# nv-tlabs/ChronoEdit

Hardware: AMD Instinct MI355X
Metric: denoising-steps/sec (higher is better)
Workload: dtype bf16

## Files before the change

chronoedit_amd/csrc/ce_common.h:

```cpp
#pragma once
#include <hip/hip_runtime.h>
#include <stdint.h>

typedef __bf16 bf16;
typedef __attribute__((ext_vector_type(2))) __bf16 bf16x2;
typedef __attribute__((ext_vector_type(4))) __bf16 bf16x4;
typedef __attribute__((ext_vector_type(8))) __bf16 bf16x8;
typedef __attribute__((ext_vector_type(2))) float f32x2;
typedef __attribute__((ext_vector_type(4))) float f32x4;
typedef __attribute__((ext_vector_type(16))) float f32x16;
typedef __attribute__((ext_vector_type(4))) uint32_t u32x4;
typedef __attribute__((ext_vector_type(2))) uint32_t u32x2;

#define CE_WAVE 64

#define CE_API extern "C" __attribute__((visibility("default")))
#ifdef CE_DIAGNOSTICS
#define CE_KNOB static int
#define CE_DIAG_COUNT_EXACT(counter)                                        \
  do {                                                                      \
    if ((threadIdx.x & 63) == 0) atomicAdd(&(counter), 1ull);               \
  } while (0)
#else
#define CE_KNOB static constexpr int
// ... 7 lines not shown

#define CE_MAX_DEVICES 16
inline int ce_device_slot() {
  int d = 0;
  if (hipGetDevice(&d) != hipSuccess || d < 0 || d >= CE_MAX_DEVICES) d = 0;
  return d;
}

inline int ce_device_cus() {
  static int cus_[CE_MAX_DEVICES] = {};
  int& cus = cus_[ce_device_slot()];
  if (cus == 0) {
    int dev = 0, n = 0;
    cus = (hipGetDevice(&dev) == hipSuccess && hipDeviceGetAttribute(&n, hipDeviceAttributeMultiprocessorCount, dev) == hipSuccess && n > 0) ? n : 256;
  }
  return cus;
}

inline int ce_split_k(int tail, int kt, int cus, long long slab_bytes, long long ws_bytes) {
  if (tail <= 0) return 1;
  for (int s = cus / tail < 8 ? cus / tail : 8; s >= 2; --s)
    if (kt % (2 * s) == 0 && tail * s * slab_bytes <= ws_bytes) return s;
  return 1;
}

inline uint32_t ce_seg_magic(int seg_k, int bk, int kt) {
  if (seg_k <= 0 || seg_k % bk) return 0;
  const int tps = seg_k / bk;
  const uint32_t magic = 65536u / (uint32_t)tps + 1u;
  for (int t = 0; t < kt; ++t)
    if ((int)((uint32_t)t * magic >> 16) != t / tps) return 0;
  return magic;
}

__device__ __forceinline__ float bf16_bits_to_f32(uint32_t bits16) { return __uint_as_float(bits16 << 16); }
__device__ __forceinline__ float bf16lo(uint32_t packed) { return __uint_as_float(packed << 16); }
__device__ __forceinline__ float bf16hi(uint32_t packed) { return __uint_as_float(packed & 0xffff0000u); }

__device__ __forceinline__ uint32_t pack_bf16(float lo, float hi) {
  f32x2 v = {lo, hi};
  bf16x2 r = __builtin_convertvector(v, bf16x2);
  return __builtin_bit_cast(uint32_t, r);
}
__device__ __forceinline__ float round_bf16(float x) {
  bf16 b = (bf16)x;
  return (float)b;
// ... 60 lines not shown
```

chronoedit_amd/csrc/ce_gemm.hip:

```cpp
#include <cmath>

#include "ce_common.h"

#define EPI_BIAS 0
#define EPI_BIAS_GELU 1
#define EPI_GATE_RES 2
#define EPI_BIAS_GELU_ERF 3
#define EPI_F32 4
#define EPI_BIAS_ROW 6
#define EPI_BIAS_T 7
#define EPI_MUL 5

namespace {

constexpr int BM = 128, BN = 128, BK = 64;
constexpr int TILE_BYTES = BM * BK * 2;
constexpr int LDC_BYTES = BN * 2 + 16;

__device__ __forceinline__ int swz_chunk(int row, int chunk) { return chunk ^ ((row >> 1) & 7); }

template <int EPI>
__global__ __launch_bounds__(256) void gemm_bf16_128(const bf16* __restrict__ A, const bf16* __restrict__ W,
                                                     bf16* __restrict__ C, const float* __restrict__ bias,
                                                     const float* __restrict__ gate, const bf16* __restrict__ res, int M,
// ... 179 lines not shown
                                 hipStream_t stream);

extern "C" void ce_gemm256_set_staggered(int on);
extern "C" int ce_gemm384_launch(const void* A, const void* W, void* C, const float* bias, int epilogue, const float* gate,
                                 const void* res, int M, int N, int K, int lda, int ldw, int ldc, int ldres, int gate_rows, int res_rows,
                                 int a_seg_k, long long a_seg_stride, int w_seg_k, long long w_seg_stride, float* ws, size_t ws_bytes,
                                 hipStream_t stream);
extern "C" int ce_gemm288_launch(const void* A, const void* W, void* C, const float* bias, int epilogue, const float* gate,
                                 const void* res, int M, int N, int K, int lda, int ldw, int ldc, int ldres, int gate_rows, int res_rows,
                                 int a_seg_k, long long a_seg_stride, int w_seg_k, long long w_seg_stride, float* ws, size_t ws_bytes,
                                 hipStream_t stream);
extern "C" int ce_gemm256w4_launch(const void* A, const void* W, void* C, const float* bias, int epilogue, const float* gate,
                                   const void* res, int M, int N, int K, int lda, int ldw, int ldc, int ldres, int gate_rows, int res_rows,
                                   int a_seg_k, long long a_seg_stride, int w_seg_k, long long w_seg_stride, int nsa, float* ws,
                                   size_t ws_bytes, hipStream_t stream);

CE_KNOB g_gemm_variant = -1;
#ifdef CE_DIAGNOSTICS
CE_API int ce_set_gemm_variant(int v) {
  const int old = g_gemm_variant;
  g_gemm_variant = v;
  ce_gemm256_set_staggered(v == 2);
  return old;
}
#endif

CE_API int ce_gemm_bf16_tile_rows(int M, int N, int K, int cus, long long ws_bytes) {
  if (M <= 0 || N <= 0 || K < 64 || cus <= 0) return 0;
  const int kt = K / 64;
  auto cost = [&](int bm) -> double {
    const long long nwg = (long long)((M + bm - 1) / bm) * ((N + 255) / 256);
    const long long full = nwg / cus;
    const int tail = (int)(nwg % cus);
    const double llc = (double)M * K * 2.0 > 128.0 * 1048576.0 ? 1.04 : 1.0;
    const double c = bm == 256 ? 1.40 : bm == 288 ? 1.40 * 1.125 * 0.985 * llc : 1.40 * 1.5 * 0.96 * llc;
    double t = (double)full * kt * c;
    if (tail > 0) {
      const int split = ce_split_k(tail, kt, cus, bm * 256 * (long long)sizeof(float), ws_bytes);
      if (split > 1) t += (double)kt / split * c + (double)tail * split * bm * 256.0 * 8.0 / 6.0e6;
      else t += (double)kt * c * pow((double)tail / cus, 0.3);
    }
    return t;
  };
  const double c384 = cost(384), c256 = cost(256);
  if (M % 288 == 0) {
    const long long nwg = (long long)(M / 288) * ((N + 255) / 256);
// ... 112 lines not shown
```

chronoedit_amd/csrc/ce_gemm256w4.hip:

```cpp
#include "ce_common.h"
#include "ce_gemm_epi.h"

namespace {

constexpr int BM = 256, BN = 256, BK = 64;
constexpr int TILE = 256 * BK * 2;
constexpr int CROW = BN * 2 + 16;
constexpr int QROW = 128 * 2 + 16;

typedef __attribute__((address_space(3))) void lds_void;

#define W4_VM(N) asm volatile("s_waitcnt vmcnt(" #N ")" ::: "memory")
#define W4_LGKM0() asm volatile("s_waitcnt lgkmcnt(0)" ::: "memory")
#define W4_BAR() __builtin_amdgcn_s_barrier()
#define W4_PIN() __builtin_amdgcn_sched_barrier(0)

__device__ __forceinline__ void tile_origin_w4(int wg, int tiles_m, int tiles_n, int bn, int& m0, int& n0) {
  constexpr int GROUP = 4;
  const int group_sz = GROUP * tiles_n;
  const int gid = wg / group_sz;
  const int first_m = gid * GROUP;
  const int gm = min(tiles_m - first_m, GROUP);
  m0 = (first_m + (wg % group_sz) % gm) * BM;
  n0 = ((wg % group_sz) / gm) * bn;
}

template <int NG>
struct FragSet {
  bf16x8 a[8], b[NG];
};

#define W4_MMA(F, G, S)                                                                                                      \
  if ((G) < NG) {                                                                                                            \
    if constexpr (REGEPI)                                                                                                    \
      asm volatile("v_mfma_f32_16x16x32_bf16 %0, %1, %2, %0" : "+a"(acc[F][(G) < NG ? (G) : 0]) : "v"((S).a[F]), "v"((S).b[(G) < NG ? (G) : 0])); \
    else                                                                                                                     \
      asm volatile("v_mfma_f32_16x16x32_bf16 %0, %1, %2, %0" : "+a"(acc[F][(G) < NG ? (G) : 0]) : "v"((S).b[(G) < NG ? (G) : 0]), "v"((S).a[F])); \
  }

template <int EPI, int NSA, bool ONEBAR, bool SEG2 = false, int NG = 8>
__global__ __launch_bounds__(256) __attribute__((amdgpu_waves_per_eu(1, 1))) void gemm_bf16_w4(
    const bf16* __restrict__ A, const bf16* __restrict__ W, bf16* __restrict__ C, const float* __restrict__ bias,
    const float* __restrict__ gate, const bf16* __restrict__ res, int M, int N, int K, int lda, int ldw, int ldc, int ldres,
    int gate_rows, int res_rows, int tiles_m, int tiles_n, int t_full, int split, float* __restrict__ ws, uint32_t a_seg_magic,
    uint32_t a_seg_extra, uint32_t w_seg_magic, uint32_t w_seg_extra, uint32_t a_seg2_magic, uint32_t a_seg2_extra) {
  extern __shared__ __attribute__((aligned(16))) unsigned char smem[];
  constexpr int BN = 32 * NG;
  constexpr bool REGEPI = NG == 8;
  constexpr int NW = NG;
  constexpr int WTILE = BN * BK * 2;
  constexpr int CROW = BN * 2 + 16;
  constexpr int W_RING = NSA * TILE;
  const int tid = threadIdx.x, lane = tid & 63;
  const int wave = __builtin_amdgcn_readfirstlane(tid >> 6);
  const int wm = wave >> 1, wn = wave & 1;
  const int fr = lane & 15, fg = lane >> 4;

  const bool partial = (int)blockIdx.x >= t_full;
  int wg, kt0 = 0, ktn = K / BK;
  if (!partial) {
    wg = xcd_remap(blockIdx.x, t_full);
  } else {
    const int tb = blockIdx.x - t_full;
    wg = t_full + tb / split;
    ktn = ktn / split;
    kt0 = (tb % split) * ktn;
  }
  int m0, n0;
  tile_origin_w4(wg, tiles_m, tiles_n, BN, m0, n0);
  const int kt_last = ktn - 1;

  uint32_t a_voff[8], w_voff[8];
#pragma unroll
  for (int p = 0; p < 8; ++p) {
    const int row = 8 * (wave + 4 * p) + (lane >> 3);
    const int chunk = (lane & 7) ^ ((row >> 1) & 7);
    a_voff[p] = (uint32_t)min(m0 + row, M - 1) * (uint32_t)(lda * 2) + chunk * 16;
    const int wrow = REGEPI ? ((row & 128) | ((row & 15) << 3) | ((row & 127) >> 4)) : row;
    w_voff[p] = (uint32_t)min(n0 + wrow, N - 1) * (uint32_t)(ldw * 2) + chunk * 16;
  }
  const auto a_rsrc = __builtin_amdgcn_make_buffer_rsrc((void*)A, 0, 0xffffffffu, 0x00020000);
  const auto w_rsrc = __builtin_amdgcn_make_buffer_rsrc((void*)W, 0, 0xffffffffu, 0x00020000);
  auto koff = [&](int t, uint32_t magic, uint32_t extra) __attribute__((always_inline)) -> int {
    const int ta = kt0 + min(t, kt_last);
    return ta * (BK * 2) + (int)((((uint32_t)ta * magic) >> 16) * extra);
  };
  auto koff_a = [&](int t) __attribute__((always_inline)) -> int {
    int o = koff(t, a_seg_magic, a_seg_extra);
    if (SEG2) o += (int)((((uint32_t)(kt0 + min(t, kt_last)) * a_seg2_magic) >> 16) * a_seg2_extra);
    return o;
  };
  auto dma_a = [&](int p, int stage_bytes, int soff) __attribute__((always_inline)) {
    __builtin_amdgcn_raw_ptr_buffer_load_lds(a_rsrc, (lds_void*)(smem + stage_bytes + (wave + 4 * p) * 1024), 16, a_voff[p], soff, 0, 0);
  };
  auto dma_w = [&](int p, int stage_bytes, int soff) __attribute__((always_inline)) {
    if (p < NW)
      __builtin_amdgcn_raw_ptr_buffer_load_lds(w_rsrc, (lds_void*)(smem + W_RING + stage_bytes + (wave + 4 * p) * 1024), 16, w_voff[p < NW ? p : 0], soff, 0, 0);
  };

  int a_rd[2], w_rd[2];
#pragma unroll
  for (int ks = 0; ks < 2; ++ks) {
    a_rd[ks] = (wm * 128 + fr) * 128 + (((fg + 4 * ks) ^ (fr >> 1)) << 4);
    w_rd[ks] = W_RING + (wn * (BN / 2) + fr) * 128 + (((fg + 4 * ks) ^ (fr >> 1)) << 4);
  }
  auto read_frag = [&](int r, int a_stage_bytes, int w_stage_bytes, FragSet<NG>& k0, FragSet<NG>& k1) __attribute__((always_inline)) {
    FragSet<NG>& s = (r >> 4) ? k1 : k0;
    const int ks = r >> 4, f = r & 7;
    if (((r >> 3) & 1) == 0)
      s.a[f] = *reinterpret_cast<const bf16x8*>(smem + a_rd[ks] + a_stage_bytes + f * 2048);
    else if (f < NG)
      s.b[f < NG ? f : 0] = *reinterpret_cast<const bf16x8*>(smem + w_rd[ks] + w_stage_bytes + f * 2048);
  };

  f32x4 acc[8][NG];
#pragma unroll
  for (int f = 0; f < 8; ++f)
#pragma unroll
    for (int g = 0; g < NG; ++g) acc[f][g] = f32x4{0.f, 0.f, 0.f, 0.f};

  {
    const int a0 = koff_a(0), w0 = koff(0, w_seg_magic, w_seg_extra);
    const int a1 = koff_a(1), w1 = koff(1, w_seg_magic, w_seg_extra);
#pragma unroll
    for (int p = 0; p < 8; ++p) dma_a(p, 0, a0);
#pragma unroll
    for (int p = 0; p < 8; ++p) dma_w(p, 0, w0);
#pragma unroll
    for (int p = 0; p < 8; ++p) dma_a(p, TILE, a1);
#pragma unroll
    for (int p = 0; p < 8; ++p) dma_w(p, WTILE, w1);
    if (NSA == 3 && !ONEBAR) {
      const int a2 = koff_a(2);
#pragma unroll
      for (int p = 0; p < 8; ++p) dma_a(p, 2 * TILE, a2);
    }
  }
  if (NSA == 3 && !ONEBAR) W4_VM(24); else if (NG == 8) W4_VM(16); else if (NG == 4) W4_VM(12); else W4_VM(11);
  W4_BAR();
  FragSet<NG> s0, s1, s2;
#pragma unroll
  for (int r = 0; r < 32; ++r) read_frag(r, 0, 0, s0, s1);
  W4_LGKM0();
  W4_PIN();

  int a_st = 0;
#define W4_TILE(T, WP, K0, K1, KN)                                                                              \
  {                                                                                                             \
    const int a_next = (a_st + TILE == NSA * TILE) ? 0 : a_st + TILE;                                          \
    const int a_nn = (a_next + TILE == NSA * TILE) ? 0 : a_next + TILE;                                        \
    const int wsoff = koff((T) + 2, w_seg_magic, w_seg_extra);                                                 \
    const int asoff = koff_a((T) + (ONEBAR ? 2 : NSA));                                                        \
    const int a_dst = ONEBAR ? a_nn : a_st;                                                                     \
    if (!ONEBAR) W4_BAR();                                                                                      \
    W4_UNIT0(0, K0, WP, wsoff) W4_UNIT0(1, K0, WP, wsoff) W4_UNIT0(2, K0, WP, wsoff) W4_UNIT0(3, K0, WP, wsoff) \
    W4_UNIT0(4, K0, WP, wsoff) W4_UNIT0(5, K0, WP, wsoff) W4_UNIT0(6, K0, WP, wsoff) W4_UNIT0(7, K0, WP, wsoff) \
    if (NSA == 3 && !ONEBAR) W4_VM(16); else if (NG == 8) W4_VM(8); else if (NG == 4) W4_VM(4); else W4_VM(3);   \
    W4_BAR();                                                                                                   \
    W4_UNIT1(0, K1, K0, KN, WP) W4_UNIT1(1, K1, K0, KN, WP) W4_UNIT1(2, K1, K0, KN, WP) W4_UNIT1(3, K1, K0, KN, WP) \
    W4_UNIT1(4, K1, K0, KN, WP) W4_UNIT1(5, K1, K0, KN, WP) W4_UNIT1(6, K1, K0, KN, WP) W4_UNIT1(7, K1, K0, KN, WP) \
    W4_LGKM0();                                                                                                 \
    W4_PIN();                                                                                                   \
    a_st = a_next;                                                                                              \
  }
#define W4_UNIT0(F, K0, WP, WSOFF)                                                                                 \
  W4_MMA(F, 0, K0);                                                                                                \
  if (ONEBAR) dma_a(F, a_dst, asoff); else dma_w(F, (WP) * WTILE, WSOFF);                                          \
  W4_PIN();                                                                                                        \
  W4_MMA(F, 1, K0); W4_MMA(F, 2, K0); W4_MMA(F, 3, K0); W4_MMA(F, 4, K0); W4_MMA(F, 5, K0); W4_MMA(F, 6, K0);      \
  W4_MMA(F, 7, K0); W4_PIN();
#define W4_UNIT1(F, K1, K0, KN, WP)                                                                                \
  W4_MMA(F, 0, K1);                                                                                                \
  if (ONEBAR) dma_w(F, (WP) * WTILE, wsoff); else dma_a(F, a_dst, asoff);                                          \
  W4_PIN();                                                                                                        \
  W4_MMA(F, 1, K1); W4_PIN();                                                                                      \
  W4_MMA(F, 2, K1); read_frag(4 * (F) + 0, a_next, (1 - (WP)) * WTILE, K0, KN); W4_PIN();                           \
  W4_MMA(F, 3, K1); read_frag(4 * (F) + 1, a_next, (1 - (WP)) * WTILE, K0, KN); W4_PIN();                           \
  W4_MMA(F, 4, K1); read_frag(4 * (F) + 2, a_next, (1 - (WP)) * WTILE, K0, KN); W4_PIN();                           \
  W4_MMA(F, 5, K1); read_frag(4 * (F) + 3, a_next, (1 - (WP)) * WTILE, K0, KN); W4_PIN();                           \
  W4_MMA(F, 6, K1); W4_MMA(F, 7, K1); W4_PIN();

  const int npairs = ktn >> 1;
  for (int it = 0; it < npairs; ++it) {
    const int t = 2 * it;
    W4_TILE(t, 0, s0, s1, s2)
    W4_TILE(t + 1, 1, s0, s2, s1)
  }
#undef W4_TILE
#undef W4_UNIT0
#undef W4_UNIT1
  W4_VM(0);
  W4_LGKM0();
  asm volatile("s_nop 15\n\ts_nop 15" ::: "memory");
  static_assert(NG == 8 || ((NG == 4 || NG == 3) && NSA == 2 && !ONEBAR), "the 256 x 128 / 256 x 96 tiles exist for the two-stage loop only");
  if constexpr (REGEPI) {
    const int col0 = n0 + wn * 128 + fr * 8;
    const bool col_ok = col0 < N;
    const int colc = min(col0, N - 8);
    const int row_base = m0 + wm * 128 + fg * 4;
    if (partial) {
      float* slab = ws + (size_t)(blockIdx.x - t_full) * (BM * BN);
#pragma unroll
      for (int f = 0; f < 8; ++f) {
        f32x4 av[8];
#pragma unroll
        for (int g = 0; g < 8; ++g) {
          asm volatile("" : "+a"(acc[f][g]));
          av[g] = acc[f][g];
        }
#pragma unroll
        for (int jj = 0; jj < 4; ++jj)
#pragma unroll
          for (int h = 0; h < 2; ++h) {
            const f32x4 o = {av[4 * h + 0][jj], av[4 * h + 1][jj], av[4 * h + 2][jj], av[4 * h + 3][jj]};
            const int lane_o = fg * 4 + jj + 16 * (2 * (fr & 1) + h);
            *reinterpret_cast<f32x4*>(slab + (((wave * 64 + f * 8 + (fr >> 1)) * 64) + lane_o) * 4) = o;
          }
      }
      return;
    }
    f32x4 bvv[2];
#pragma unroll
    for (int h = 0; h < 2; ++h)
      bvv[h] = (EPI != EPI_BIAS_ROW && bias != nullptr) ? *reinterpret_cast<const f32x4*>(bias + colc + 4 * h) : f32x4{0.f, 0.f, 0.f, 0.f};
    const auto c_rsrc = __builtin_amdgcn_make_buffer_rsrc((void*)C, 0, (uint32_t)(M - 1) * (uint32_t)(ldc * 2) + (uint32_t)N * 2u, 0x00020000);
    f32x4 gA[2], gB[2];
    int g_switch = 0x7fffffff;
    u32x4 rv[8][4];
    if (EPI == EPI_GATE_RES) {
      gA[0] = gA[1] = gB[0] = gB[1] = f32x4{1.f, 1.f, 1.f, 1.f};
      if (gate != nullptr) {
        const int s0 = gate_rows > 0 ? m0 / gate_rows : 0;
        const int s1 = gate_rows > 0 ? min(M - 1, m0 + BM - 1) / gate_rows : 0;
        const float* ga = gate + (size_t)s0 * N + colc;
        const float* gb = gate + (size_t)s1 * N + colc;
        gA[0] = *reinterpret_cast<const f32x4*>(ga);
        gA[1] = *reinterpret_cast<const f32x4*>(ga + 4);
        gB[0] = *reinterpret_cast<const f32x4*>(gb);
        gB[1] = *reinterpret_cast<const f32x4*>(gb + 4);
        if (s1 != s0) g_switch = s1 * gate_rows;
      }
#pragma unroll
      for (int f = 0; f < 8; ++f)
#pragma unroll
        for (int jj = 0; jj < 4; ++jj)
          rv[f][jj] = *reinterpret_cast<const u32x4*>(res + (size_t)res_row(min(row_base + f * 16 + jj, M - 1), res_wrap(m0, res_rows)) * ldres + colc);
    }
#pragma unroll
    for (int f = 0; f < 8; ++f) {
      f32x4 av[8];
#pragma unroll
      for (int g = 0; g < 8; ++g) {
        asm volatile("" : "+a"(acc[f][g]));
        av[g] = acc[f][g];
      }
      f32x4 brow4 = {0.f, 0.f, 0.f, 0.f};
      if (EPI == EPI_BIAS_ROW) brow4 = *reinterpret_cast<const f32x4*>(bias + min(row_base + f * 16, M - 4));
#pragma unroll
      for (int jj = 0; jj < 4; ++jj) {
        const int m = row_base + f * 16 + jj;
        u32x4 y;
#pragma unroll
        for (int q = 0; q < 4; ++q) {
          const int h = q >> 1, e = 2 * (q & 1);
          const float b0 = EPI == EPI_BIAS_ROW ? brow4[jj] : bvv[h][e], b1 = EPI == EPI_BIAS_ROW ? brow4[jj] : bvv[h][e + 1];
          y[q] = pack_bf16(av[2 * q][jj] + b0, av[2 * q + 1][jj] + b1);
        }
        u32x4 o = y;
        if (EPI == EPI_BIAS_GELU) {
#pragma unroll
          for (int q = 0; q < 4; ++q) o[q] = pack_bf16(gelu_tanh(bf16lo(y[q])), gelu_tanh(bf16hi(y[q])));
        } else if (EPI == EPI_BIAS_GELU_ERF) {
// ... 108 lines not shown
        const u32x4 r = rv[p][tt];
        u32x4 o;
#pragma unroll
        for (int q = 0; q < 4; ++q) {
          const float ga = q < 2 ? g0[2 * q] : g1[2 * q - 4], gb = q < 2 ? g0[2 * q + 1] : g1[2 * q - 3];
          o[q] = pack_bf16(mul_then_add(bf16lo(y[q]), ga, bf16lo(r[q])), mul_then_add(bf16hi(y[q]), gb, bf16hi(r[q])));
        }
        const uint32_t coff = (m < M && my_n < N) ? (uint32_t)m * (uint32_t)(ldc * 2) + (uint32_t)my_n * 2u : 0xffffffffu;
        __builtin_amdgcn_raw_buffer_store_b128(o, c_rsrc, coff, 0, 0);
      }
    } else if (EPI != EPI_GATE_RES) {
      epi_chunks<EPI, CH>(smem, CROW,
                         [&](int tt, int& rl, int& cc, int& mr) {
                           bool ok;
                           rl = chunk_row(tt, ok);
                           cc = my_cc;
                           mr = ok ? (rl >> 5) * 128 + p * 32 + (rl & 31) : (1 << 28);
                         },
                         m0, n0, C, gate, res, M, N, ldc, ldres, gate_rows, res_rows);
    }
  }
}

template <int EPI>
__global__ __launch_bounds__(256) void gemm256w4_reduce(bf16* __restrict__ C, const float* __restrict__ bias, const float* __restrict__ gate,
                                                        const bf16* __restrict__ res, int M, int N, int ldc, int ldres, int gate_rows, int res_rows,
                                                        int tiles_m, int tiles_n, int t_full, int split, const float* __restrict__ ws) {
  extern __shared__ __attribute__((aligned(16))) unsigned char smem[];
  const int tid = threadIdx.x, lane = tid & 63, w = tid >> 6;
  const int fr = lane & 15, fg = lane >> 4;
  const int tile = blockIdx.x >> 2, q = blockIdx.x & 3;
  int m0, n0;
  tile_origin_w4(t_full + tile, tiles_m, tiles_n, BN, m0, n0);
  m0 += (q >> 1) * 128;
  n0 += (q & 1) * 128;
  const float* slab = ws + (size_t)tile * split * (BM * BN);
#pragma unroll
  for (int ff = 0; ff < 2; ++ff) {
    const int f = 2 * w + ff;
    const int rl = f * 16 + fr;
    float brow = 0.f;
    if (EPI == EPI_BIAS_ROW) brow = bias[min(m0 + rl, M - 1)];
#pragma unroll
    for (int g = 0; g < 8; ++g) {
      const int cl = g * 16 + fg * 4;
      f32x4 bv = (EPI != EPI_BIAS_ROW && bias != nullptr) ? *reinterpret_cast<const f32x4*>(bias + min(n0 + cl, N - 4)) : f32x4{0.f, 0.f, 0.f, 0.f};
      if (EPI == EPI_BIAS_ROW) bv[0] = bv[1] = bv[2] = bv[3] = brow;
      const int e = (((q * 64 + f * 8 + g) * 64) + lane) * 4;
      f32x4 v = *reinterpret_cast<const f32x4*>(slab + e);
      for (int sidx = 1; sidx < split; ++sidx) v += *reinterpret_cast<const f32x4*>(slab + (size_t)sidx * (BM * BN) + e);
      const u32x2 pk = {pack_bf16(v[0] + bv[0], v[1] + bv[1]), pack_bf16(v[2] + bv[2], v[3] + bv[3])};
      *reinterpret_cast<u32x2*>(smem + rl * QROW + cl * 2) = pk;
    }
  }
  __syncthreads();
  epi_chunks<EPI, 8>(smem, QROW, [&](int tt, int& rl, int& cc, int& mr) { const int c = tid + 256 * tt; rl = mr = c >> 4; cc = c & 15; }, m0, n0,
                     C, gate, res, M, N, ldc, ldres, gate_rows, res_rows);
}

}

extern "C" int ce_gemm256_launch(const void* A, const void* W, void* C, const float* bias, int epilogue, const float* gate,
// ... 20 lines not shown
  const int tiles_m = (M + BM - 1) / BM, tiles_n = (N + bn - 1) / bn;
  const int nwg = tiles_m * tiles_n, kt = K / BK;
  uint32_t a_seg_magic = 0, a_seg_extra = 0, w_seg_magic = 0, w_seg_extra = 0;
  auto seg = [&](int seg_k, long long seg_stride, uint32_t& magic, uint32_t& extra_out) -> int {
    if (seg_k <= 0 || seg_k >= K) return CE_OK;
    magic = ce_seg_magic(seg_k, BK, kt);
    const long long extra = (seg_stride - seg_k) * 2;
    if (!magic || extra < 0 || extra * ((K + seg_k - 1) / seg_k) + (long long)K * 2 >= (1ll << 31)) return CE_ERR_SHAPE;
    extra_out = (uint32_t)extra;
    return CE_OK;
  };
  if (int rc = seg(a_seg_k, a_seg_stride, a_seg_magic, a_seg_extra)) return rc;
  if (int rc = seg(w_seg_k, w_seg_stride, w_seg_magic, w_seg_extra)) return rc;
  uint32_t a_seg2_magic = 0, a_seg2_extra = 0;
  if (seg2 && a_seg2_k < K) {
    a_seg2_magic = ce_seg_magic(a_seg2_k, BK, kt);
    if (!a_seg2_magic) return CE_ERR_SHAPE;
    const long long extra = (a_seg2_stride - (long long)(a_seg2_k / a_seg_k) * a_seg_stride) * 2;
    const long long reach = ((long long)(K - 1) / a_seg2_k) * a_seg2_stride * 2 + (long long)(a_seg2_k / a_seg_k) * a_seg_stride * 2 + (long long)a_seg_k * 2;
    if (extra < 0 || reach >= (1ll << 31)) return CE_ERR_SHAPE;
    a_seg2_extra = (uint32_t)extra;
  }
  const int cus = ce_device_cus();
  int tail = nwg % cus;
  const int split = seg2 ? 1 : ce_split_k(tail, kt, cus, BM * BN * sizeof(float), ws ? (long long)ws_bytes : 0);
  if (split == 1) tail = 0;
  const int t_full2 = nwg - tail;
  dim3 grid(t_full2 + tail * split), block(256);
  const int lds3 = 5 * TILE, lds2 = 4 * TILE;
  if (seg2) {
    const int lds2n = 2 * TILE + 2 * (128 * BK * 2);
    const int lds2m = 2 * TILE + 2 * (96 * BK * 2);
    static bool seg2_done_[CE_MAX_DEVICES] = {};
    bool& seg2_done = seg2_done_[ce_device_slot()];
    if (!seg2_done) {
      if (hipFuncSetAttribute((const void*)gemm_bf16_w4<EPI_BIAS, 2, false, true>, hipFuncAttributeMaxDynamicSharedMemorySize, lds2) != hipSuccess ||
          hipFuncSetAttribute((const void*)gemm_bf16_w4<EPI_GATE_RES, 2, false, true>, hipFuncAttributeMaxDynamicSharedMemorySize, lds2) != hipSuccess ||
          hipFuncSetAttribute((const void*)gemm_bf16_w4<EPI_BIAS, 2, false, true, 4>, hipFuncAttributeMaxDynamicSharedMemorySize, lds2n) != hipSuccess ||
          hipFuncSetAttribute((const void*)gemm_bf16_w4<EPI_GATE_RES, 2, false, true, 4>, hipFuncAttributeMaxDynamicSharedMemorySize, lds2n) != hipSuccess ||
          hipFuncSetAttribute((const void*)gemm_bf16_w4<EPI_BIAS, 2, false, true, 3>, hipFuncAttributeMaxDynamicSharedMemorySize, lds2m) != hipSuccess ||
          hipFuncSetAttribute((const void*)gemm_bf16_w4<EPI_GATE_RES, 2, false, true, 3>, hipFuncAttributeMaxDynamicSharedMemorySize, lds2m) != hipSuccess)
        return CE_ERR_ARG;
      seg2_done = true;
    }
#define CE_LAUNCH_SEG2(E, NGV, LDS)                                                                                                     \
  hipLaunchKernelGGL((gemm_bf16_w4<E, 2, false, true, NGV>), grid, block, LDS, stream, (const bf16*)A, (const bf16*)W, (bf16*)C, bias, gate, \
                     (const bf16*)res, M, N, K, lda, ldw, ldc, ldres, gate_rows, res_rows, tiles_m, tiles_n, t_full2, split, ws, a_seg_magic,   \
                     a_seg_extra, w_seg_magic, w_seg_extra, a_seg2_magic, a_seg2_extra)
    if (epilogue == EPI_BIAS) {
      if (ng == 8) CE_LAUNCH_SEG2(EPI_BIAS, 8, lds2); else if (ng == 4) CE_LAUNCH_SEG2(EPI_BIAS, 4, lds2n); else CE_LAUNCH_SEG2(EPI_BIAS, 3, lds2m);
    } else {
      if (ng == 8) CE_LAUNCH_SEG2(EPI_GATE_RES, 8, lds2); else if (ng == 4) CE_LAUNCH_SEG2(EPI_GATE_RES, 4, lds2n); else CE_LAUNCH_SEG2(EPI_GATE_RES, 3, lds2m);
    }
#undef CE_LAUNCH_SEG2
    return (int)hipGetLastError();
  }
  static bool attr_done_[CE_MAX_DEVICES][8] = {};
  bool* attr_done = attr_done_[ce_device_slot()];
#define CE_LAUNCH(E)                                                                                                       \
  do {                                                                                                                     \
    if (!attr_done[E]) {                                                                                                   \
      if (hipFuncSetAttribute((const void*)gemm_bf16_w4<E, 3, false>, hipFuncAttributeMaxDynamicSharedMemorySize, lds3) != hipSuccess) return CE_ERR_ARG; \
      if (hipFuncSetAttribute((const void*)gemm_bf16_w4<E, 3, true>, hipFuncAttributeMaxDynamicSharedMemorySize, lds3) != hipSuccess) return CE_ERR_ARG; \
      if (hipFuncSetAttribute((const void*)gemm_bf16_w4<E, 2, false>, hipFuncAttributeMaxDynamicSharedMemorySize, lds2) != hipSuccess) return CE_ERR_ARG; \
      (void)hipFuncSetAttribute((const void*)gemm256w4_reduce<E>, hipFuncAttributeMaxDynamicSharedMemorySize, 128 * QROW); \
      attr_done[E] = true;                                                                                                 \
    }                                                                                                                      \
    if (nsa == 1)                                                                                                          \
      hipLaunchKernelGGL((gemm_bf16_w4<E, 3, true>), grid, block, lds3, stream, (const bf16*)A, (const bf16*)W, (bf16*)C, bias, gate, \
                         (const bf16*)res, M, N, K, lda, ldw, ldc, ldres, gate_rows, res_rows, tiles_m, tiles_n, t_full2, split, ws, \
                         a_seg_magic, a_seg_extra, w_seg_magic, w_seg_extra, 0u, 0u);                                      \
    else if (nsa == 3)                                                                                                     \
      hipLaunchKernelGGL((gemm_bf16_w4<E, 3, false>), grid, block, lds3, stream, (const bf16*)A, (const bf16*)W, (bf16*)C, bias, gate, \
                         (const bf16*)res, M, N, K, lda, ldw, ldc, ldres, gate_rows, res_rows, tiles_m, tiles_n, t_full2, split, ws, \
                         a_seg_magic, a_seg_extra, w_seg_magic, w_seg_extra, 0u, 0u);                                      \
    else                                                                                                                   \
      hipLaunchKernelGGL((gemm_bf16_w4<E, 2, false>), grid, block, lds2, stream, (const bf16*)A, (const bf16*)W, (bf16*)C, bias, gate, \
                         (const bf16*)res, M, N, K, lda, ldw, ldc, ldres, gate_rows, res_rows, tiles_m, tiles_n, t_full2, split, ws, \
                         a_seg_magic, a_seg_extra, w_seg_magic, w_seg_extra, 0u, 0u);                                      \
    if (tail)                                                                                                              \
      hipLaunchKernelGGL((gemm256w4_reduce<E>), dim3(4 * tail), block, 128 * QROW, stream, (bf16*)C, bias, gate,           \
                         (const bf16*)res, M, N, ldc, ldres, gate_rows, res_rows, tiles_m, tiles_n, t_full2, split, ws);           \
  } while (0)
  switch (epilogue) {
    case EPI_BIAS: CE_LAUNCH(EPI_BIAS); break;
    case EPI_BIAS_GELU: CE_LAUNCH(EPI_BIAS_GELU); break;
    case EPI_GATE_RES: CE_LAUNCH(EPI_GATE_RES); break;
    case EPI_BIAS_GELU_ERF: CE_LAUNCH(EPI_BIAS_GELU_ERF); break;
    case EPI_BIAS_ROW: CE_LAUNCH(EPI_BIAS_ROW); break;
    default: return CE_ERR_ARG;
  }
#undef CE_LAUNCH
  return (int)hipGetLastError();
}

extern "C" int ce_gemm256w4_launch(const void* A, const void* W, void* C, const float* bias, int epilogue, const float* gate,
                                   const void* res, int M, int N, int K, int lda, int ldw, int ldc, int ldres, int gate_rows, int res_rows,
                                   int a_seg_k, long long a_seg_stride, int w_seg_k, long long w_seg_stride, int nsa, float* ws,
                                   size_t ws_bytes, hipStream_t stream) {
  return w4_launch(A, W, C, bias, epilogue, gate, res, M, N, K, lda, ldw, ldc, ldres, gate_rows, res_rows, a_seg_k, a_seg_stride, w_seg_k, w_seg_stride,
                   0, 0, nsa, 8, ws, ws_bytes, stream);
}

extern "C" int ce_gemm256w4_seg2_launch(const void* A, const void* W, void* C, const float* bias, int epilogue, const void* res, int M, int N,
                                        int K, int lda, int ldw, int ldc, int ldres, int a_seg_k, long long a_seg_stride, int a_seg2_k,
// ... 29 lines not shown
```

chronoedit_amd/hiplib.py:

```python
from __future__ import annotations

import ctypes
import os
import re
import subprocess
from typing import Dict, List

PKG_DIR = os.path.dirname(os.path.abspath(__file__))
ROOT = os.path.dirname(PKG_DIR)
CSRC = os.path.join(PKG_DIR, "csrc")
LIB_DIR = os.path.join(PKG_DIR, "lib")
LIB_PATH = os.path.join(LIB_DIR, "libchronoedit_hip.so")
DIAG_LIB_PATH = os.path.join(LIB_DIR, "libchronoedit_hip_diag.so")
OBJ_DIR = os.path.join(LIB_DIR, "obj")
HEADER = os.path.join(ROOT, "include", "chronoedit_hip.h")
DIAG_HEADER = os.path.join(ROOT, "include", "chronoedit_hip_diag.h")

DIAG_SOURCES = ["ce_gemm.hip", "ce_gemm256.hip", "ce_attn.hip", "ce_attn_fp8.hip", "ce_gemm_fp8.hip", "ce_gemm_fp8w4.hip"]
DIAG_ONLY_SOURCES = ["ce_attn16.hip"]
SOURCES = ["ce_rowops.hip", "ce_gemm.hip", "ce_gemm256.hip", "ce_gemm256w4.hip", "ce_gemm384.hip", "ce_attn.hip", "ce_attn16.hip", "ce_attn_fp8.hip", "ce_sched.hip", "ce_conv.hip", "ce_enc.hip", "ce_gemm_fp8.hip", "ce_gemm_fp8w4.hip", "ce_comm.hip", "ce_lora.hip", "ce_tea.hip", "ce_image.hip", "ce_region.hip", "ce_sparse.hip", "ce_region_auto.hip", "ce_focus.hip", "ce_autofocus.hip", "ce_preview.hip", "ce_lift.hip", "ce_sketch.hip", "ce_components.hip"]

_c = ctypes
_P, _I, _F = _c.c_void_p, _c.c_int, _c.c_float

# ... 82 lines not shown
    "ce_preview_rgb_u8": [_P, _P, _P, _P, _P, _I, _I, _I, _I, _I, _I, _I, _P],
    "ce_preview_gram_f64": [_P, _I, _P, _I, _P, _P, _c.c_size_t, _I, _I, _I, _I, _P],
    "ce_lift_fit_q16": [_P, _P, _P, _I, _I, _I, _I, _I, _F, _P],
    "ce_lift_smooth_f32": [_P, _P, _P, _P, _P, _I, _I, _I, _I, _P],
    "ce_lift_gate_f32": [_P, _P, _I, _I, _I, _I, _F, _F, _P],
    "ce_lift_apply_u8": [_P, _P, _P, _P, _P, _P, _P, _P, _P, _P, _I, _I, _I, _I, _I, _P],
    "ce_sketch_changed_u8": [_P, _P, _P, _c.c_longlong, _I, _P],
    "ce_sketch_dilate_u8": [_P, _P, _I, _I, _I, _I, _P, _c.c_size_t, _P],
    "ce_sketch_box_u8": [_P, _P, _I, _I, _I, _I, _P, _c.c_size_t, _P],
    "ce_components_roots_i32": [_P, _P, _I, _I, _P],
    "ce_components_sums_i32": [_P, _P, _P, _I, _I, _P],
    "ce_components_keep_u8": [_P, _P, _P, _P, _P, _I, _I, _I, _I, _I, _P],
    "ce_components_seeds_f32": [_P, _P, _P, _I, _P],
    "ce_components_masked_f32": [_P, _P, _P, _I, _P],
    "ce_build_info": [],
}
DIAG_SIGNATURES: Dict[str, List] = {
    "ce_set_gemm_variant": [_I],
    "ce_set_attention_waves": [_I],
    "ce_set_gemm_fp8_variant": [_I],
    "ce_set_attention_mxfp8_variant": [_I],
    "ce_set_attention_mxfp8_persistent": [_I],
    "ce_diag_attention_exact_route_hits": [_P, _I],
}


def header_symbols(diag: bool = False) -> List[str]:
    txt = open(DIAG_HEADER if diag else HEADER).read()
    return re.findall(r"^int (ce_\w+)\(", txt, flags=re.M)


def exported_symbols(path: str) -> List[str]:
    nm = "/opt/rocm/lib/llvm/bin/llvm-nm" if os.path.exists("/opt/rocm/lib/llvm/bin/llvm-nm") else "nm"
    out = subprocess.run([nm, "-D", "--defined-only", path], check=True, capture_output=True, text=True).stdout
    return sorted(l.split()[-1] for l in out.splitlines() if l.split() and l.split()[-2] in ("T", "t", "W", "D", "B"))


HIPCC_FLAGS = ["--offload-arch=gfx950", "-O3", "-std=c++17", "-fPIC", "-fvisibility=hidden"]


def build(force: bool = False, verbose: bool = False, jobs: int = 0) -> str:
    import glob
    from concurrent.futures import ThreadPoolExecutor
    srcs = [s for s in SOURCES if os.path.exists(os.path.join(CSRC, s))]
    hdrs = sorted(glob.glob(os.path.join(CSRC, "*.h"))) + [HEADER, DIAG_HEADER]
    hdr_m = max(os.path.getmtime(d) for d in hdrs)
# ... 89 lines not shown
```

include/chronoedit_hip_diag.h:

```cpp
#ifndef CHRONOEDIT_HIP_DIAG_H
#define CHRONOEDIT_HIP_DIAG_H

#include "chronoedit_hip.h"

#ifdef __cplusplus
extern "C" {
#endif

int ce_set_gemm_variant(int variant);

int ce_set_attention_waves(int nwave);

int ce_set_gemm_fp8_variant(int variant);

int ce_set_attention_mxfp8_variant(int variant);

int ce_set_attention_mxfp8_persistent(int n);

int ce_diag_attention_exact_route_hits(unsigned long long* hits, int reset);

#ifdef __cplusplus
}
#endif
#endif
```

Before: 3.126.

## Specialize w4 GEMM ragged M-tail tiles with short-row bodies and tail planning

Splits the w4 GEMM kernel into a tile body templated on the number of active 16-row fragments. When the last M tile holds few valid rows, it runs a shortened body that skips the MFMAs, LDS reads and epilogue rows that are entirely out of range. Adds a tail planner that, for a small ragged M remainder, can skip split-K and let the short tail tiles fill idle CUs in the last wave. The reduce kernel and the XCD remap are updated to handle the partial final M tile. This grows code size and adds template instances, and the gain depends on M not being a multiple of 256.

```diff
diff --git a/chronoedit_amd/csrc/ce_common.h b/chronoedit_amd/csrc/ce_common.h
--- a/chronoedit_amd/csrc/ce_common.h
+++ b/chronoedit_amd/csrc/ce_common.h
@@ -53,6 +53,22 @@
   for (int s = cus / tail < 8 ? cus / tail : 8; s >= 2; --s)
     if (kt % (2 * s) == 0 && tail * s * slab_bytes <= ws_bytes) return s;
   return 1;
+}
+
+struct CeTailPlan {
+  int tail, split;
+};
+inline CeTailPlan ce_gemm256w4_tail_plan(int M, int tiles_n, int kt, int cus, long long ws_bytes) {
+  const long long whole = (long long)(M / 256) * tiles_n, nwg = (long long)((M + 255) / 256) * tiles_n;
+  const int r = M % 256, p = r > 128 ? 8 : (r + 15) / 16 < 4 ? 4 : (r + 15) / 16;
+  if (r > 0 && p < 8) {
+    const long long rem = whole % cus, rounds = (whole + cus - 1) / cus;
+    if (rem > 0 && tiles_n <= (cus - rem) * (8 / p) && rounds <= nwg / cus) return {0, 1};
+  }
+  int tail = (int)(nwg % cus);
+  const int split = ce_split_k(tail, kt, cus, 256 * 256 * (long long)sizeof(float), ws_bytes);
+  if (split == 1) tail = 0;
+  return {tail, split};
 }
 
 inline uint32_t ce_seg_magic(int seg_k, int bk, int kt) {
diff --git a/chronoedit_amd/csrc/ce_gemm.hip b/chronoedit_amd/csrc/ce_gemm.hip
--- a/chronoedit_amd/csrc/ce_gemm.hip
+++ b/chronoedit_amd/csrc/ce_gemm.hip
@@ -225,6 +225,16 @@
   g_gemm_variant = v;
   ce_gemm256_set_staggered(v == 2);
   return old;
+}
+CE_API int ce_diag_gemm256w4_plan(int M, int N, int K, int cus, long long ws_bytes, int* plan) {
+  if (M <= 0 || N <= 0 || K < 64 || cus <= 0 || !plan) return CE_ERR_ARG;
+  const int tiles_n = (N + 255) / 256;
+  const CeTailPlan p = ce_gemm256w4_tail_plan(M, tiles_n, K / 64, cus, ws_bytes);
+  plan[0] = p.tail;
+  plan[1] = p.split;
+  plan[2] = (M + 255) / 256 * tiles_n - p.tail + p.tail * p.split;
+  plan[3] = M % 256 ? tiles_n : 0;
+  return CE_OK;
 }
 #endif
 
diff --git a/chronoedit_amd/csrc/ce_gemm256w4.hip b/chronoedit_amd/csrc/ce_gemm256w4.hip
--- a/chronoedit_amd/csrc/ce_gemm256w4.hip
+++ b/chronoedit_amd/csrc/ce_gemm256w4.hip
@@ -17,6 +17,11 @@
 
 __device__ __forceinline__ void tile_origin_w4(int wg, int tiles_m, int tiles_n, int bn, int& m0, int& n0) {
   constexpr int GROUP = 4;
+  if (wg >= tiles_m * tiles_n) {
+    m0 = tiles_m * BM;
+    n0 = (wg - tiles_m * tiles_n) * bn;
+    return;
+  }
   const int group_sz = GROUP * tiles_n;
   const int gid = wg / group_sz;
   const int first_m = gid * GROUP;
@@ -38,13 +43,17 @@
       asm volatile("v_mfma_f32_16x16x32_bf16 %0, %1, %2, %0" : "+a"(acc[F][(G) < NG ? (G) : 0]) : "v"((S).b[(G) < NG ? (G) : 0]), "v"((S).a[F])); \
   }
 
-template <int EPI, int NSA, bool ONEBAR, bool SEG2 = false, int NG = 8>
-__global__ __launch_bounds__(256) __attribute__((amdgpu_waves_per_eu(1, 1))) void gemm_bf16_w4(
+template <int EPI, int NSA, bool ONEBAR, bool SEG2, int NG, int RF>
+__device__ __forceinline__ void w4_tile(
     const bf16* __restrict__ A, const bf16* __restrict__ W, bf16* __restrict__ C, const float* __restrict__ bias,
-    const float* __restrict__ gate, const bf16* __restrict__ res, int M, int N, int K, int lda, int ldw, int ldc, int ldres,
-    int gate_rows, int res_rows, int tiles_m, int tiles_n, int t_full, int split, float* __restrict__ ws, uint32_t a_seg_magic,
-    uint32_t a_seg_extra, uint32_t w_seg_magic, uint32_t w_seg_extra, uint32_t a_seg2_magic, uint32_t a_seg2_extra) {
+    const float* __restrict__ gate, const bf16* __restrict__ res, int M, int N, int lda, int ldw, int ldc, int ldres,
+    int gate_rows, int res_rows, int t_full, float* __restrict__ ws, uint32_t a_seg_magic,
+    uint32_t a_seg_extra, uint32_t w_seg_magic, uint32_t w_seg_extra, uint32_t a_seg2_magic, uint32_t a_seg2_extra, int m0, int n0, int kt0,
+    int ktn, bool partial) {
   extern __shared__ __attribute__((aligned(16))) unsigned char smem[];
+  static_assert(RF == 16 || (NG == 8 && RF >= 1 && RF <= 4), "short bodies: the register-direct epilogue only");
+  constexpr int RFW = RF == 16 ? 8 : RF;
+  constexpr int WROWS = 16 * RFW;
   constexpr int BN = 32 * NG;
   constexpr bool REGEPI = NG == 8;
   constexpr int NW = NG;
@@ -56,18 +65,6 @@
   const int wm = wave >> 1, wn = wave & 1;
   const int fr = lane & 15, fg = lane >> 4;
 
-  const bool partial = (int)blockIdx.x >= t_full;
-  int wg, kt0 = 0, ktn = K / BK;
-  if (!partial) {
-    wg = xcd_remap(blockIdx.x, t_full);
-  } else {
-    const int tb = blockIdx.x - t_full;
-    wg = t_full + tb / split;
-    ktn = ktn / split;
-    kt0 = (tb % split) * ktn;
-  }
-  int m0, n0;
-  tile_origin_w4(wg, tiles_m, tiles_n, BN, m0, n0);
   const int kt_last = ktn - 1;
 
   uint32_t a_voff[8], w_voff[8];
@@ -101,21 +98,22 @@
   int a_rd[2], w_rd[2];
 #pragma unroll
   for (int ks = 0; ks < 2; ++ks) {
-    a_rd[ks] = (wm * 128 + fr) * 128 + (((fg + 4 * ks) ^ (fr >> 1)) << 4);
+    a_rd[ks] = (wm * WROWS + fr) * 128 + (((fg + 4 * ks) ^ (fr >> 1)) << 4);
     w_rd[ks] = W_RING + (wn * (BN / 2) + fr) * 128 + (((fg + 4 * ks) ^ (fr >> 1)) << 4);
   }
-  auto read_frag = [&](int r, int a_stage_bytes, int w_stage_bytes, FragSet<NG>& k0, FragSet<NG>& k1) __attribute__((always_inline)) {
+  auto read_frag = [&](int r, int a_stage_bytes, int w_stage_bytes, FragSet<NG>& k0, FragSet<NG>& k1, int rf) __attribute__((always_inline)) {
     FragSet<NG>& s = (r >> 4) ? k1 : k0;
     const int ks = r >> 4, f = r & 7;
-    if (((r >> 3) & 1) == 0)
-      s.a[f] = *reinterpret_cast<const bf16x8*>(smem + a_rd[ks] + a_stage_bytes + f * 2048);
-    else if (f < NG)
-      s.b[f < NG ? f : 0] = *reinterpret_cast<const bf16x8*>(smem + w_rd[ks] + w_stage_bytes + f * 2048);
+    if (((r >> 3) & 1) == 0) {
+      if (f < rf) s.a[f] = *reinterpret_cast<const bf16x8*>(smem + a_rd[ks] + a_stage_bytes + f * 2048);
+    } else if (f < NG) {
+      if (rf > 0) s.b[f < NG ? f : 0] = *reinterpret_cast<const bf16x8*>(smem + w_rd[ks] + w_stage_bytes + f * 2048);
+    }
   };
 
   f32x4 acc[8][NG];
 #pragma unroll
-  for (int f = 0; f < 8; ++f)
+  for (int f = 0; f < RFW; ++f)
 #pragma unroll
     for (int g = 0; g < NG; ++g) acc[f][g] = f32x4{0.f, 0.f, 0.f, 0.f};
 
@@ -139,10 +137,6 @@
   if (NSA == 3 && !ONEBAR) W4_VM(24); else if (NG == 8) W4_VM(16); else if (NG == 4) W4_VM(12); else W4_VM(11);
   W4_BAR();
   FragSet<NG> s0, s1, s2;
-#pragma unroll
-  for (int r = 0; r < 32; ++r) read_frag(r, 0, 0, s0, s1);
-  W4_LGKM0();
-  W4_PIN();
 
   int a_st = 0;
 #define W4_TILE(T, WP, K0, K1, KN)                                                                              \
@@ -164,28 +158,41 @@
     a_st = a_next;                                                                                              \
   }
 #define W4_UNIT0(F, K0, WP, WSOFF)                                                                                 \
-  W4_MMA(F, 0, K0);                                                                                                \
+  if constexpr ((F) < rf) { W4_MMA(F, 0, K0); }                                                                    \
   if (ONEBAR) dma_a(F, a_dst, asoff); else dma_w(F, (WP) * WTILE, WSOFF);                                          \
   W4_PIN();                                                                                                        \
-  W4_MMA(F, 1, K0); W4_MMA(F, 2, K0); W4_MMA(F, 3, K0); W4_MMA(F, 4, K0); W4_MMA(F, 5, K0); W4_MMA(F, 6, K0);      \
-  W4_MMA(F, 7, K0); W4_PIN();
+  if constexpr ((F) < rf) {                                                                                        \
+    W4_MMA(F, 1, K0); W4_MMA(F, 2, K0); W4_MMA(F, 3, K0); W4_MMA(F, 4, K0); W4_MMA(F, 5, K0); W4_MMA(F, 6, K0);    \
+    W4_MMA(F, 7, K0);                                                                                              \
+  }                                                                                                                \
+  W4_PIN();
 #define W4_UNIT1(F, K1, K0, KN, WP)                                                                                \
-  W4_MMA(F, 0, K1);                                                                                                \
+  if constexpr ((F) < rf) { W4_MMA(F, 0, K1); }                                                                    \
   if (ONEBAR) dma_w(F, (WP) * WTILE, wsoff); else dma_a(F, a_dst, asoff);                                          \
   W4_PIN();                                                                                                        \
-  W4_MMA(F, 1, K1); W4_PIN();                                                                                      \
-  W4_MMA(F, 2, K1); read_frag(4 * (F) + 0, a_next, (1 - (WP)) * WTILE, K0, KN); W4_PIN();                           \
-  W4_MMA(F, 3, K1); read_frag(4 * (F) + 1, a_next, (1 - (WP)) * WTILE, K0, KN); W4_PIN();                           \
-  W4_MMA(F, 4, K1); read_frag(4 * (F) + 2, a_next, (1 - (WP)) * WTILE, K0, KN); W4_PIN();                           \
-  W4_MMA(F, 5, K1); read_frag(4 * (F) + 3, a_next, (1 - (WP)) * WTILE, K0, KN); W4_PIN();                           \
-  W4_MMA(F, 6, K1); W4_MMA(F, 7, K1); W4_PIN();
+  if constexpr ((F) < rf) { W4_MMA(F, 1, K1); } W4_PIN();                                                          \
+  if constexpr ((F) < rf) { W4_MMA(F, 2, K1); } read_frag(4 * (F) + 0, a_next, (1 - (WP)) * WTILE, K0, KN, rf); W4_PIN();     \
+  if constexpr ((F) < rf) { W4_MMA(F, 3, K1); } read_frag(4 * (F) + 1, a_next, (1 - (WP)) * WTILE, K0, KN, rf); W4_PIN();     \
+  if constexpr ((F) < rf) { W4_MMA(F, 4, K1); } read_frag(4 * (F) + 2, a_next, (1 - (WP)) * WTILE, K0, KN, rf); W4_PIN();     \
+  if constexpr ((F) < rf) { W4_MMA(F, 5, K1); } read_frag(4 * (F) + 3, a_next, (1 - (WP)) * WTILE, K0, KN, rf); W4_PIN();     \
+  if constexpr ((F) < rf) { W4_MMA(F, 6, K1); W4_MMA(F, 7, K1); } W4_PIN();
+#define W4_LOOP()                          \
+  for (int it = 0; it < npairs; ++it) {    \
+    const int t = 2 * it;                  \
+    W4_TILE(t, 0, s0, s1, s2)              \
+    W4_TILE(t + 1, 1, s0, s2, s1)          \
+  }
 
   const int npairs = ktn >> 1;
-  for (int it = 0; it < npairs; ++it) {
-    const int t = 2 * it;
-    W4_TILE(t, 0, s0, s1, s2)
-    W4_TILE(t + 1, 1, s0, s2, s1)
-  }
+  {
+    constexpr int rf = RFW;
+#pragma unroll
+    for (int r = 0; r < 32; ++r) read_frag(r, 0, 0, s0, s1, rf);
+    W4_LGKM0();
+    W4_PIN();
+    W4_LOOP()
+  }
+#undef W4_LOOP
 #undef W4_TILE
 #undef W4_UNIT0
 #undef W4_UNIT1
@@ -197,11 +204,11 @@
     const int col0 = n0 + wn * 128 + fr * 8;
     const bool col_ok = col0 < N;
     const int colc = min(col0, N - 8);
-    const int row_base = m0 + wm * 128 + fg * 4;
+    const int row_base = m0 + wm * WROWS + fg * 4;
     if (partial) {
       float* slab = ws + (size_t)(blockIdx.x - t_full) * (BM * BN);
 #pragma unroll
-      for (int f = 0; f < 8; ++f) {
+      for (int f = 0; f < RFW; ++f) {
         f32x4 av[8];
 #pragma unroll
         for (int g = 0; g < 8; ++g) {
@@ -214,7 +221,8 @@
           for (int h = 0; h < 2; ++h) {
             const f32x4 o = {av[4 * h + 0][jj], av[4 * h + 1][jj], av[4 * h + 2][jj], av[4 * h + 3][jj]};
             const int lane_o = fg * 4 + jj + 16 * (2 * (fr & 1) + h);
-            *reinterpret_cast<f32x4*>(slab + (((wave * 64 + f * 8 + (fr >> 1)) * 64) + lane_o) * 4) = o;
+            const int F = wm * RFW + f;
+            *reinterpret_cast<f32x4*>(slab + ((((2 * (F >> 3) + wn) * 64 + (F & 7) * 8 + (fr >> 1)) * 64) + lane_o) * 4) = o;
           }
       }
       return;
@@ -226,7 +234,7 @@
     const auto c_rsrc = __builtin_amdgcn_make_buffer_rsrc((void*)C, 0, (uint32_t)(M - 1) * (uint32_t)(ldc * 2) + (uint32_t)N * 2u, 0x00020000);
     f32x4 gA[2], gB[2];
     int g_switch = 0x7fffffff;
-    u32x4 rv[8][4];
+    u32x4 rv[RFW][4];
     if (EPI == EPI_GATE_RES) {
       gA[0] = gA[1] = gB[0] = gB[1] = f32x4{1.f, 1.f, 1.f, 1.f};
       if (gate != nullptr) {
@@ -241,13 +249,13 @@
         if (s1 != s0) g_switch = s1 * gate_rows;
       }
 #pragma unroll
-      for (int f = 0; f < 8; ++f)
+      for (int f = 0; f < RFW; ++f)
 #pragma unroll
         for (int jj = 0; jj < 4; ++jj)
           rv[f][jj] = *reinterpret_cast<const u32x4*>(res + (size_t)res_row(min(row_base + f * 16 + jj, M - 1), res_wrap(m0, res_rows)) * ldres + colc);
     }
 #pragma unroll
-    for (int f = 0; f < 8; ++f) {
+    for (int f = 0; f < RFW; ++f) {
       f32x4 av[8];
 #pragma unroll
       for (int g = 0; g < 8; ++g) {
@@ -402,6 +410,41 @@
   }
 }
 
+template <int EPI, int NSA, bool ONEBAR, bool SEG2 = false, int NG = 8>
+__global__ __launch_bounds__(256) __attribute__((amdgpu_waves_per_eu(1, 1))) void gemm_bf16_w4(
+    const bf16* __restrict__ A, const bf16* __restrict__ W, bf16* __restrict__ C, const float* __restrict__ bias,
+    const float* __restrict__ gate, const bf16* __restrict__ res, int M, int N, int K, int lda, int ldw, int ldc, int ldres,
+    int gate_rows, int res_rows, int tiles_n, int t_full, int split, float* __restrict__ ws, uint32_t a_seg_magic,
+    uint32_t a_seg_extra, uint32_t w_seg_magic, uint32_t w_seg_extra, uint32_t a_seg2_magic, uint32_t a_seg2_extra) {
+  const bool partial = (int)blockIdx.x >= t_full;
+  const int tiles_mw = M / BM, n_remap = min(t_full, tiles_mw * tiles_n);
+  int wg, kt0 = 0, ktn = K / BK;
+  if (!partial) {
+    wg = (int)blockIdx.x < n_remap ? xcd_remap(blockIdx.x, n_remap) : (int)blockIdx.x;
+  } else {
+    const int tb = blockIdx.x - t_full;
+    wg = t_full + tb / split;
+    ktn = ktn / split;
+    kt0 = (tb % split) * ktn;
+  }
+  int m0, n0;
+  tile_origin_w4(wg, tiles_mw, tiles_n, 32 * NG, m0, n0);
+#define W4_BODY(RF)                                                                                                                       \
+  w4_tile<EPI, NSA, ONEBAR, SEG2, NG, RF>(A, W, C, bias, gate, res, M, N, lda, ldw, ldc, ldres, gate_rows, res_rows, t_full, ws, a_seg_magic, \
+                                          a_seg_extra, w_seg_magic, w_seg_extra, a_seg2_magic, a_seg2_extra, m0, n0, kt0, ktn, partial)
+  const int rows = M - m0;
+  if constexpr (NG != 8) {
+    W4_BODY(16);
+  } else {
+    if (__builtin_expect(rows > 128, 1)) W4_BODY(16);
+    else if (rows > 96) W4_BODY(4);
+    else if (rows > 64) W4_BODY(3);
+    else if (rows > 32) W4_BODY(2);
+    else W4_BODY(1);
+  }
+#undef W4_BODY
+}
+
 template <int EPI>
 __global__ __launch_bounds__(256) void gemm256w4_reduce(bf16* __restrict__ C, const float* __restrict__ bias, const float* __restrict__ gate,
                                                         const bf16* __restrict__ res, int M, int N, int ldc, int ldres, int gate_rows, int res_rows,
@@ -414,10 +457,12 @@
   tile_origin_w4(t_full + tile, tiles_m, tiles_n, BN, m0, n0);
   m0 += (q >> 1) * 128;
   n0 += (q & 1) * 128;
+  if (m0 >= M) return;
   const float* slab = ws + (size_t)tile * split * (BM * BN);
 #pragma unroll
   for (int ff = 0; ff < 2; ++ff) {
     const int f = 2 * w + ff;
+    if (m0 + f * 16 >= M) break;
     const int rl = f * 16 + fr;
     float brow = 0.f;
     if (EPI == EPI_BIAS_ROW) brow = bias[min(m0 + rl, M - 1)];
@@ -484,9 +529,8 @@
     a_seg2_extra = (uint32_t)extra;
   }
   const int cus = ce_device_cus();
-  int tail = nwg % cus;
-  const int split = seg2 ? 1 : ce_split_k(tail, kt, cus, BM * BN * sizeof(float), ws ? (long long)ws_bytes : 0);
-  if (split == 1) tail = 0;
+  const CeTailPlan plan = seg2 ? CeTailPlan{0, 1} : ce_gemm256w4_tail_plan(M, tiles_n, kt, cus, ws ? (long long)ws_bytes : 0);
+  const int tail = plan.tail, split = plan.split;
   const int t_full2 = nwg - tail;
   dim3 grid(t_full2 + tail * split), block(256);
   const int lds3 = 5 * TILE, lds2 = 4 * TILE;
@@ -507,7 +551,7 @@
     }
 #define CE_LAUNCH_SEG2(E, NGV, LDS)                                                                                                     \
   hipLaunchKernelGGL((gemm_bf16_w4<E, 2, false, true, NGV>), grid, block, LDS, stream, (const bf16*)A, (const bf16*)W, (bf16*)C, bias, gate, \
-                     (const bf16*)res, M, N, K, lda, ldw, ldc, ldres, gate_rows, res_rows, tiles_m, tiles_n, t_full2, split, ws, a_seg_magic,   \
+                     (const bf16*)res, M, N, K, lda, ldw, ldc, ldres, gate_rows, res_rows, tiles_n, t_full2, split, ws, a_seg_magic,   \
                      a_seg_extra, w_seg_magic, w_seg_extra, a_seg2_magic, a_seg2_extra)
     if (epilogue == EPI_BIAS) {
       if (ng == 8) CE_LAUNCH_SEG2(EPI_BIAS, 8, lds2); else if (ng == 4) CE_LAUNCH_SEG2(EPI_BIAS, 4, lds2n); else CE_LAUNCH_SEG2(EPI_BIAS, 3, lds2m);
@@ -530,19 +574,19 @@
     }                                                                                                                      \
     if (nsa == 1)                                                                                                          \
       hipLaunchKernelGGL((gemm_bf16_w4<E, 3, true>), grid, block, lds3, stream, (const bf16*)A, (const bf16*)W, (bf16*)C, bias, gate, \
-                         (const bf16*)res, M, N, K, lda, ldw, ldc, ldres, gate_rows, res_rows, tiles_m, tiles_n, t_full2, split, ws, \
+                         (const bf16*)res, M, N, K, lda, ldw, ldc, ldres, gate_rows, res_rows, tiles_n, t_full2, split, ws, \
                          a_seg_magic, a_seg_extra, w_seg_magic, w_seg_extra, 0u, 0u);                                      \
     else if (nsa == 3)                                                                                                     \
       hipLaunchKernelGGL((gemm_bf16_w4<E, 3, false>), grid, block, lds3, stream, (const bf16*)A, (const bf16*)W, (bf16*)C, bias, gate, \
-                         (const bf16*)res, M, N, K, lda, ldw, ldc, ldres, gate_rows, res_rows, tiles_m, tiles_n, t_full2, split, ws, \
+                         (const bf16*)res, M, N, K, lda, ldw, ldc, ldres, gate_rows, res_rows, tiles_n, t_full2, split, ws, \
                          a_seg_magic, a_seg_extra, w_seg_magic, w_seg_extra, 0u, 0u);                                      \
     else                                                                                                                   \
       hipLaunchKernelGGL((gemm_bf16_w4<E, 2, false>), grid, block, lds2, stream, (const bf16*)A, (const bf16*)W, (bf16*)C, bias, gate, \
-                         (const bf16*)res, M, N, K, lda, ldw, ldc, ldres, gate_rows, res_rows, tiles_m, tiles_n, t_full2, split, ws, \
+                         (const bf16*)res, M, N, K, lda, ldw, ldc, ldres, gate_rows, res_rows, tiles_n, t_full2, split, ws, \
                          a_seg_magic, a_seg_extra, w_seg_magic, w_seg_extra, 0u, 0u);                                      \
     if (tail)                                                                                                              \
       hipLaunchKernelGGL((gemm256w4_reduce<E>), dim3(4 * tail), block, 128 * QROW, stream, (bf16*)C, bias, gate,           \
-                         (const bf16*)res, M, N, ldc, ldres, gate_rows, res_rows, tiles_m, tiles_n, t_full2, split, ws);           \
+                         (const bf16*)res, M, N, ldc, ldres, gate_rows, res_rows, M / BM, tiles_n, t_full2, split, ws);            \
   } while (0)
   switch (epilogue) {
     case EPI_BIAS: CE_LAUNCH(EPI_BIAS); break;
diff --git a/chronoedit_amd/hiplib.py b/chronoedit_amd/hiplib.py
--- a/chronoedit_amd/hiplib.py
+++ b/chronoedit_amd/hiplib.py
@@ -128,6 +128,7 @@
     "ce_set_attention_mxfp8_variant": [_I],
     "ce_set_attention_mxfp8_persistent": [_I],
     "ce_diag_attention_exact_route_hits": [_P, _I],
+    "ce_diag_gemm256w4_plan": [_I, _I, _I, _I, _c.c_longlong, _P],
 }
 
 
diff --git a/include/chronoedit_hip_diag.h b/include/chronoedit_hip_diag.h
--- a/include/chronoedit_hip_diag.h
+++ b/include/chronoedit_hip_diag.h
@@ -19,6 +19,8 @@
 
 int ce_diag_attention_exact_route_hits(unsigned long long* hits, int reset);
 
+int ce_diag_gemm256w4_plan(int M, int N, int K, int cus, long long ws_bytes, int* plan);
+
 #ifdef __cplusplus
 }
 #endif
```

New measurement: 3.128 (median of 2 runs). Within noise of the previous version (+0.1%).
